# NVIDIA/DeepLearningExamples

Measured on AMD Instinct MI355X. Metric: training samples/sec, higher is better.
Workload: dtype bf16; 1 GPU; ResNet-50 v1.5 (PyTorch/Classification/ConvNets) synthetic ImageNet 224x224, label smoothing 0.1, SGD momentum 0.875 (BASELINE.json configs[1]); batch_per_gpu=256, global_batch=256, layout=NHWC, hip_graph=False, parallelism=single GPU

## Files before the change

### deeplearningexamples_amd/csrc/conv3x3.hip

```cpp
#include "gemm_tiles.h"

#define C3_MT 256

struct C3Args {
  const unsigned short* x;
  const unsigned short* w;
  unsigned short* y;
  float* stats;
  int N, H, W, CI, CO;
  int Wp, IMG, G;
  int tiles_m, tiles_n, pieces;
  FastDiv dIMG, dWp;
  const float* scale;
  const float* shift;
  const unsigned short* residual;
  int relu;
};

template <int DT, bool DGRAD, int NT, bool AFF = false>
__global__ __launch_bounds__(256, 2) void conv3x3_kernel(C3Args p) {
  constexpr int WTN = NT / 32;
  typedef Loader<DGRAD ? 1 : 0, NT, 4> LB;
  extern __shared__ __attribute__((aligned(16))) unsigned char smem_raw[];
  unsigned short* patch = (unsigned short*)smem_raw;
  unsigned short* bst = patch + p.pieces * 512;
  const int tid = threadIdx.x, lane = tid & 63, wave = tid >> 6;
  const int fr = lane & 31, fh = lane >> 5;

  int bid = blockIdx.x;
  {
    const int ntiles = p.tiles_m * p.tiles_n;
    const int q = ntiles >> 3, r = ntiles & 7, xcd = bid & 7, loc = bid >> 3;
    bid = (xcd < r ? xcd * (q + 1) : r * (q + 1) + (xcd - r) * q) + loc;
  }
  const int tm = bid / p.tiles_n, tn = bid - tm * p.tiles_n;
  const int g0 = tm * C3_MT, n0 = tn * NT;
  const int f0 = g0 - p.Wp - 1;

  ConvGeom nog;
  nog.H = nog.W = nog.C = nog.P = nog.Q = nog.R = nog.S = nog.stride = nog.Ko = 1; nog.pad = 0;
  LB lb;
  const long long ldb = 9LL * (DGRAD ? p.CO : p.CI);
  lb.init(wave, lane, n0, p.CO, ldb, nog);

  auto issue_patch = [&](int cc) __attribute__((always_inline)) {
    __amdgpu_buffer_rsrc_t rs = __builtin_amdgcn_make_buffer_rsrc((void*)p.x, 0, 0xFFFFFFE0, 0x00020000);
    for (int pc = wave; pc < p.pieces; pc += 4) {
      const int slot = pc * 8 + (lane >> 3), chunk = (lane & 7) ^ swz_kc(slot);
      const int f = f0 + slot;
      const int fc = f < 0 ? 0 : f;
      const int n = fd_div(fc, p.dIMG), rem = fc - n * p.IMG;
      const int hp = fd_div(rem, p.dWp), wp = rem - hp * p.Wp;
      const bool ok = f >= 0 && f < p.G && hp >= 1 && wp >= 1 && wp <= p.W;
      const unsigned off = (unsigned)(((((long long)n * p.H + (hp - 1)) * p.W + (wp - 1)) * p.CI + cc * 64 + chunk * 8) * 2);
      dma16(rs, patch + pc * 512, ok ? off : OOB_OFF);
    }
  };
  auto issue_b = [&](int cc, int tap, int stage) __attribute__((always_inline)) {
    const unsigned short* base = DGRAD ? p.w + (long long)cc * 64 * ldb + (8 - tap) * p.CO + n0
                                       : p.w + (long long)n0 * ldb + tap * p.CI + cc * 64;
    lb.template issue<0, LB::NP>(base, bst + stage * (NT * 64), wave, 64, 0, nog);
  };

  float16_t acc[2][WTN];
#pragma unroll
  for (int i = 0; i < 2; ++i)
#pragma unroll
    for (int j = 0; j < WTN; ++j)
#pragma unroll
      for (int r = 0; r < 16; ++r) acc[i][j][r] = 0.f;

  const int nchunks = p.CI >> 6;
  issue_patch(0);
  issue_b(0, 0, 0);
  int stage = 0;
  for (int cc = 0; cc < nchunks; ++cc) {
    if (cc > 0) {
      __syncthreads();
      issue_patch(cc);
    }
    int tapoff = 0, tapcol = 0;
    for (int tap = 0; tap < 9; ++tap) {
      __builtin_amdgcn_s_waitcnt(0x0F70);
      __syncthreads();
      if (tap < 8) issue_b(cc, tap + 1, stage ^ 1);
      else if (cc + 1 < nchunks) issue_b(cc + 1, 0, stage ^ 1);
      const unsigned short* tb = bst + stage * (NT * 64);
      int abase[2];
#pragma unroll
      for (int i = 0; i < 2; ++i) {
        const int slot = wave * 64 + i * 32 + fr + tapoff;
        abase[i] = slot * 64 + ((fh ^ swz_kc(slot)) << 3);
      }
      if constexpr (!DGRAD) {
#pragma unroll
        for (int ks = 0; ks < 4; ++ks) {
          ushort8_t fa[2], fb[WTN];
#pragma unroll
          for (int i = 0; i < 2; ++i) fa[i] = *(const ushort8_t*)(patch + (abase[i] ^ (ks << 4)));
#pragma unroll
          for (int j = 0; j < WTN; ++j) fb[j] = frag_issue<false, NT>(tb, j * 32, ks, lane);
#pragma unroll
          for (int i = 0; i < 2; ++i)
#pragma unroll
            for (int j = 0; j < WTN; ++j) acc[i][j] = Mfma32x16<DT>::run(fb[j], fa[i], acc[i][j]);
        }
      } else {
        TrPair fb[2][WTN];
#pragma unroll
        for (int j = 0; j < WTN; ++j) fb[0][j] = frag_issue<true, NT>(tb, j * 32, 0, lane);
        static_for<0, 4>([&](auto KS) __attribute__((always_inline)) {
          constexpr int ks = decltype(KS)::value, cur = ks & 1, nxt = cur ^ 1;
          ushort8_t fa[2], vb[WTN];
#pragma unroll
          for (int i = 0; i < 2; ++i) fa[i] = *(const ushort8_t*)(patch + (abase[i] ^ (ks << 4)));
          frag_wait<true>();
          if constexpr (ks < 3) {
#pragma unroll
            for (int j = 0; j < WTN; ++j) fb[nxt][j] = frag_issue<true, NT>(tb, j * 32, ks + 1, lane);
          }
#pragma unroll
          for (int j = 0; j < WTN; ++j) vb[j] = frag_value(fb[cur][j]);
#pragma unroll
          for (int i = 0; i < 2; ++i)
#pragma unroll
            for (int j = 0; j < WTN; ++j) acc[i][j] = Mfma32x16<DT>::run(vb[j], fa[i], acc[i][j]);
        });
      }
      stage ^= 1;
      if (++tapcol == 3) { tapcol = 0; tapoff += p.Wp - 2; } else ++tapoff;
    }
  }

  __syncthreads();
  constexpr int LPR = NT / 8, RPT = 64 / LPR, TRIPS = 32 / RPT, MASK = NT / 4 - 1;
  float* epi = (float*)smem_raw + wave * (32 * NT);
  const int erow = lane / LPR, ecg = lane % LPR;
  if constexpr (AFF) {
    float sc[8], sh[8];
    {
      const float4_t s0 = *(const float4_t*)(p.scale + n0 + ecg * 8), s1 = *(const float4_t*)(p.scale + n0 + ecg * 8 + 4);
      const float4_t h0 = *(const float4_t*)(p.shift + n0 + ecg * 8), h1 = *(const float4_t*)(p.shift + n0 + ecg * 8 + 4);
#pragma unroll
      for (int r = 0; r < 4; ++r) { sc[r] = s0[r]; sc[4 + r] = s1[r]; sh[r] = h0[r]; sh[4 + r] = h1[r]; }
    }
#pragma unroll
    for (int i = 0; i < 2; ++i) {
      int off[TRIPS];
      ushort8_t rv[TRIPS];
#pragma unroll
      for (int t = 0; t < TRIPS; ++t) {
        const int g = g0 + wave * 64 + i * 32 + t * RPT + erow;
        const int n = fd_div(g, p.dIMG), rem = g - n * p.IMG;
// ... 39 lines not shown
#pragma unroll
  for (int i = 0; i < 2; ++i) {
#pragma unroll
    for (int j = 0; j < WTN; ++j)
#pragma unroll
      for (int qd = 0; qd < 4; ++qd) {
        const float4_t v = {acc[i][j][qd * 4 + 0], acc[i][j][qd * 4 + 1], acc[i][j][qd * 4 + 2], acc[i][j][qd * 4 + 3]};
        const int c4 = j * 8 + qd * 2 + fh;
        *(float4_t*)(epi + fr * NT + ((c4 ^ (fr & MASK)) << 2)) = v;
      }
    asm volatile("s_waitcnt lgkmcnt(0)" ::: "memory");
#pragma unroll
    for (int t = 0; t < TRIPS; ++t) {
      const int row = t * RPT + erow;
      const float4_t lo = *(const float4_t*)(epi + row * NT + (((2 * ecg) ^ (row & MASK)) << 2));
      const float4_t hi = *(const float4_t*)(epi + row * NT + (((2 * ecg + 1) ^ (row & MASK)) << 2));
      const int g = g0 + wave * 64 + i * 32 + row;
      const int n = fd_div(g, p.dIMG), rem = g - n * p.IMG;
      const int hp = fd_div(rem, p.dWp), wp = rem - hp * p.Wp;
      const bool ok = g < p.G && hp >= 1 && wp >= 1 && wp <= p.W;
      if (ok) {
        float v[8] = {lo[0], lo[1], lo[2], lo[3], hi[0], hi[1], hi[2], hi[3]};
        const ushort8_t ov = pack8<DT>(v);
        *(ushort8_t*)(p.y + (((long long)n * p.H + (hp - 1)) * p.W + (wp - 1)) * p.CO + n0 + ecg * 8) = ov;
        if (p.stats) {
          float vr[8];
          unpack8<DT>(ov, vr);
#pragma unroll
          for (int r = 0; r < 8; ++r) { st0[r] += vr[r]; st1[r] += vr[r] * vr[r]; }
        }
      }
    }
    asm volatile("s_waitcnt lgkmcnt(0)" ::: "memory");
  }
  if (p.stats) {
#pragma unroll
    for (int r = 0; r < 8; ++r) {
#pragma unroll
      for (int o = LPR; o < 64; o <<= 1) {
        st0[r] += __shfl_xor(st0[r], o, 64);
        st1[r] += __shfl_xor(st1[r], o, 64);
      }
    }
    __syncthreads();
    float* red = (float*)smem_raw;
    if (lane < LPR) {
#pragma unroll
// ... 52 lines not shown
                               int W, int C, int Ko, int dgrad, int dtype, hipStream_t stream) {
  const int CO = dgrad ? C : Ko;
  C3Args p;
  int NT;
  size_t lds;
  if (!c3_plan(x, w, y, N, H, W, dgrad ? Ko : C, CO, dgrad, dtype, &p, &NT, &lds)) return 0;
  p.stats = stats;
  if (stats && stats_bytes < (long long)p.tiles_m * 2 * CO * 4) {
    dle_set_error("conv3x3: statistics buffer too small (%d tile rows)", p.tiles_m);
    return 2;
  }
  dim3 grid((unsigned)(p.tiles_m * p.tiles_n)), block(256);
#define C3_GO(DT, DG, NTV) DLE_LAUNCH_LDS((conv3x3_kernel<DT, DG, NTV>), grid, block, lds, stream, p)
#define C3_PICK(DT) do { if (dgrad) { if (NT == 128) C3_GO(DT, true, 128); else C3_GO(DT, true, 64); } \
                         else { if (NT == 128) C3_GO(DT, false, 128); else C3_GO(DT, false, 64); } } while (0)
  if (dtype == DLE_F16) C3_PICK(DLE_F16); else C3_PICK(DLE_BF16);
#undef C3_GO
#undef C3_PICK
  hipError_t e = hipGetLastError();
  if (e != hipSuccess) { dle_set_error("conv3x3 launch failed: %s", hipGetErrorString(e)); return (int)e + 1000; }
  return 1;
}

static long long g_c3_affine_launches = 0;
extern "C" int64_t dle_conv3x3_affine_launch_count(void) { return __atomic_load_n(&g_c3_affine_launches, __ATOMIC_RELAXED); }

extern "C" int dle_conv3x3_affine_try(const void* x, const void* w, void* y, const float* scale, const float* shift,
                                      const void* residual, int N, int H, int W, int C, int Ko, int dtype, int relu,
                                      hipStream_t stream) {
  if ((((uintptr_t)scale) | ((uintptr_t)shift) | ((uintptr_t)residual)) & 15) return 0;
  if ((long long)N * H * W * Ko >= 0x7FFFFFFFLL) return 0;
  C3Args p;
  int NT;
  size_t lds;
  if (!c3_plan(x, w, y, N, H, W, C, Ko, 0, dtype, &p, &NT, &lds)) return 0;
  p.scale = scale; p.shift = shift; p.residual = (const unsigned short*)residual; p.relu = relu;
  dim3 grid((unsigned)(p.tiles_m * p.tiles_n)), block(256);
#define C3_GO(DT, NTV) DLE_LAUNCH_LDS((conv3x3_kernel<DT, false, NTV, true>), grid, block, lds, stream, p)
#define C3_PICK(DT) do { if (NT == 128) C3_GO(DT, 128); else C3_GO(DT, 64); } while (0)
  if (dtype == DLE_F16) C3_PICK(DLE_F16); else C3_PICK(DLE_BF16);
#undef C3_GO
#undef C3_PICK
  hipError_t e = hipGetLastError();
  if (e != hipSuccess) { dle_set_error("conv3x3 affine launch failed: %s", hipGetErrorString(e)); return (int)e + 1000; }
  __atomic_fetch_add(&g_c3_affine_launches, 1, __ATOMIC_RELAXED);
  return 1;
// ... 2 lines not shown
```

### deeplearningexamples_amd/csrc/gemm_dma.hip

```cpp
#include "gemm_tiles.h"

#define SLAB_MODE(p) ((p).ws != nullptr)
#define GEMM2_LDS_BYTES (2 * (BM * BK + BN * BK) * 2)

struct Gemm2Args {
  const unsigned short* A;
  const unsigned short* B;
  void* C;
  void* aux;
  const float* bias;
  const unsigned short* mask_src;
  int M, N, K;
  long long lda, ldb, ldc;
  int out_dtype, act, splitk, accumulate;
  float alpha;
  float* ws;
  ConvGeom cg;
  int batch_inner, batch_count;
  int unused_pad;
  float* stats;
  int force_small;
  int stats_sums;
  long long row_extra;
  FastDiv row_div;
// ... 896 lines not shown
  if ((M & 255) != 0 || workspace_bytes < (long long)((M + 127) / 128) * N * 4) return 0;
  bool launched = false;
  DLE_TRY(dle_gemm8_relu_bwd_bits_try(A, B, C, bits, (float*)workspace, M, N, K, lda, ldb, dtype, stream), launched = true);
  if (!launched) return 0;
  hipLaunchKernelGGL(colsum_fold_kernel, dim3((N + 15) / 16), dim3(256), 0, stream, (const float*)workspace, colsum_out, N,
                     (M + 127) / 128, accumulate_colsum);
  hipError_t e = hipGetLastError();
  if (e != hipSuccess) { dle_set_error("colsum_fold launch failed: %s", hipGetErrorString(e)); return (int)e + 1000; }
  return 1;
}


static int conv_check(const char* what, int N, int H, int W, int C, int Ko, int R, int S, int stride, int pad,
                      int P, int Q, int dtype) {
  DLE_CHECK_ARG(dtype == DLE_F16 || dtype == DLE_BF16, "%s: 16-bit dtypes only (got %d)", what, dtype);
  DLE_CHECK_ARG(N > 0 && H > 0 && W > 0 && R > 0 && S > 0 && stride > 0 && pad >= 0, "%s: bad geometry", what);
  DLE_CHECK_ARG(C % 8 == 0 && Ko % 8 == 0, "%s: channel counts must be multiples of 8 (C=%d, K=%d)", what, C, Ko);
  DLE_CHECK_ARG(P == (H + 2 * pad - R) / stride + 1 && Q == (W + 2 * pad - S) / stride + 1, "%s: output size mismatch", what);
  DLE_CHECK_ARG((long long)N * H * W * C * 2 < 0xFFFFFFE0LL && (long long)N * P * Q * Ko * 2 < 0xFFFFFFE0LL,
                "%s: tensors above 4 GiB are not addressable by this kernel", what);
  return 0;
}

extern "C" int dle_conv2d_fwd(const void* x, const void* w, void* y, const float* bias, int N, int H, int W, int C,
                              int Ko, int R, int S, int stride, int pad, int dtype, int out_dtype, int act,
                              hipStream_t stream) {
  const int P = (H + 2 * pad - R) / stride + 1, Q = (W + 2 * pad - S) / stride + 1;
  if (int rc = conv_check("conv2d_fwd", N, H, W, C, Ko, R, S, stride, pad, P, Q, dtype)) return rc;
  DLE_CHECK_ARG(x && w && y, "conv2d_fwd: null pointer");
  DLE_CHECK_ARG(act == ACT_NONE || act == ACT_RELU, "conv2d_fwd: unsupported epilogue %d", act);
  if (R == 3 && S == 3 && stride == 1 && pad == 1 && !bias && act == ACT_NONE && out_dtype == dtype)
    DLE_TRY(dle_conv3x3_try(x, w, y, nullptr, 0, N, H, W, C, Ko, 0, dtype, stream), return 0);
  Gemm2Args p = {};
  p.A = (const unsigned short*)x; p.B = (const unsigned short*)w; p.C = y; p.bias = bias;
  p.M = N * P * Q; p.N = Ko; p.K = R * S * C; p.lda = 0; p.ldb = (long long)R * S * C; p.ldc = Ko;
  p.out_dtype = out_dtype; p.act = act; p.splitk = 1; p.accumulate = 0; p.alpha = 1.f;
  p.cg = make_geom(H, W, C, P, Q, R, S, stride, pad, Ko);
  return launch_gemm(p, dtype, 2, 0, 0, stream);
}

extern "C" int dle_conv2d_fwd_affine(const void* x, const void* w, void* y, const float* scale, const float* shift,
                                     const void* residual, int N, int H, int W, int C, int Ko, int R, int S, int stride,
                                     int pad, int dtype, int relu, hipStream_t stream) {
  DLE_CHECK_ARG(R > 0 && S > 0 && stride > 0 && pad >= 0 && H + 2 * pad >= R && W + 2 * pad >= S, "conv2d_fwd_affine: bad geometry");
  const int P = (H + 2 * pad - R) / stride + 1, Q = (W + 2 * pad - S) / stride + 1;
  if (int rc = conv_check("conv2d_fwd_affine", N, H, W, C, Ko, R, S, stride, pad, P, Q, dtype)) return rc;
  DLE_CHECK_ARG(x && w && y && scale && shift, "conv2d_fwd_affine: null pointer");
  DLE_CHECK_ARG(((((uintptr_t)x) | ((uintptr_t)w) | ((uintptr_t)y) | ((uintptr_t)scale) | ((uintptr_t)shift) | ((uintptr_t)residual)) & 15) == 0,
                "conv2d_fwd_affine: every operand must be 16-byte aligned");
  const long long M = (long long)N * P * Q;
  DLE_CHECK_ARG(M < 0x7FFFFFFFLL && (long long)R * S * C < 0x7FFFFFFFLL, "conv2d_fwd_affine: too many output pixels");
  if (R == 3 && S == 3 && stride == 1 && pad == 1)
    DLE_TRY(dle_conv3x3_affine_try(x, w, y, scale, shift, residual, N, H, W, C, Ko, dtype, relu, stream), return 0);
  const bool matrix = R == 1 && S == 1 && stride == 1 && pad == 0 && (long long)C * BM * 2 <= 0x7FFFFFFFLL;
  Gemm2Args p = {};
// ... 14 lines not shown
  if (dtype == DLE_F16) GOA(DLE_F16); else GOA(DLE_BF16);
#undef GOA
  hipError_t e = hipGetLastError();
  if (e != hipSuccess) { dle_set_error("conv2d_fwd_affine launch failed: %s", hipGetErrorString(e)); return (int)e; }
  return 0;
}

static const long long CONV_STATS_GEMM8_MAX_M = 65536;

extern "C" int dle_conv2d_fwd_colstats(const void* x, const void* w, void* y, int N, int H, int W, int C, int Ko, int R,
                                       int S, int stride, int pad, int dtype, float* col_partial,
                                       int64_t col_partial_bytes, int* groups, hipStream_t stream) {
  const int P = (H + 2 * pad - R) / stride + 1, Q = (W + 2 * pad - S) / stride + 1;
  if (int rc = conv_check("conv2d_fwd_colstats", N, H, W, C, Ko, R, S, stride, pad, P, Q, dtype)) return rc;
  DLE_CHECK_ARG(x && w && y && col_partial && groups, "conv2d_fwd_colstats: null pointer");
  DLE_CHECK_ARG((((uintptr_t)y) & 15) == 0, "conv2d_fwd_colstats: output must be 16-byte aligned");
  const long long M = (long long)N * P * Q;
  const int g = (int)((M + BM - 1) / BM);
  DLE_CHECK_ARG(col_partial_bytes >= (long long)g * 2 * Ko * 4, "conv2d_fwd_colstats: partial buffer too small (%lld tile rows)", (long long)g);
  *groups = g;
  if (R == 3 && S == 3 && stride == 1 && pad == 1 && col_partial_bytes >= (long long)dle_conv3x3_tiles(N, H, W) * 2 * Ko * 4)
    DLE_TRY(dle_conv3x3_try(x, w, y, col_partial, col_partial_bytes, N, H, W, C, Ko, 0, dtype, stream),
            *groups = (int)(((long long)N * (H + 1) * (W + 2) + 255) / 256); return 0);
  const bool plain = R == 1 && S == 1 && stride == 1 && pad == 0;
  if (plain && M < 0x7FFFFFFF && (M & 255) == 0 && M <= CONV_STATS_GEMM8_MAX_M && C >= 128 && Ko >= 256)
    DLE_TRY(dle_gemm8_colstats_try(x, w, y, (int)M, Ko, C, C, C, Ko, dtype, col_partial, stream), *groups = g; return 0);
  if (plain && M < 0x7FFFFFFF) {
    static const int kmin = dle_env_int("DLE_EXPAND_STATS_KMIN", 64);
    const int eg = dle_gemm_expand_groups((int)M, Ko, C);
    if (dle_gemm_expand_enabled() && C >= kmin && col_partial_bytes >= (long long)eg * 2 * Ko * 4)
      DLE_TRY(dle_gemm_expand_try(x, w, y, nullptr, nullptr, col_partial, (int)M, Ko, C, C, C, Ko, 1, dtype, dtype, EX_ACT_NONE, stream),
              *groups = eg; return 0);
  }
  Gemm2Args p = {};
  p.A = (const unsigned short*)x; p.B = (const unsigned short*)w; p.C = y;
  p.M = (int)M; p.N = Ko; p.K = R * S * C; p.ldb = (long long)R * S * C; p.ldc = Ko;
  p.out_dtype = dtype; p.act = ACT_NONE; p.splitk = 1; p.accumulate = 0; p.alpha = 1.f;
  p.stats = col_partial; p.force_small = 1;
  p.lda = plain ? C : 0;
  p.cg = make_geom(H, W, C, P, Q, R, S, stride, pad, Ko);
  return launch_gemm(p, dtype, plain ? 0 : 2, 0, 0, stream);
}

extern "C" int dle_conv2d_dgrad(const void* dy, const void* w, void* dx, const void* addend, int N, int H, int W,
                                int C, int Ko, int R, int S, int stride, int pad, int dtype, hipStream_t stream) {
  const int P = (H + 2 * pad - R) / stride + 1, Q = (W + 2 * pad - S) / stride + 1;
  if (int rc = conv_check("conv2d_dgrad", N, H, W, C, Ko, R, S, stride, pad, P, Q, dtype)) return rc;
  DLE_CHECK_ARG(dy && w && dx, "conv2d_dgrad: null pointer");
  if (R == 3 && S == 3 && stride == 1 && pad == 1 && !addend)
    DLE_TRY(dle_conv3x3_try(dy, w, dx, nullptr, 0, N, H, W, C, Ko, 1, dtype, stream), return 0);
  Gemm2Args p = {};
  p.A = (const unsigned short*)dy; p.B = (const unsigned short*)w; p.C = dx;
  p.mask_src = (const unsigned short*)addend;
  p.M = N * H * W; p.N = C; p.K = R * S * Ko; p.lda = 0; p.ldb = 0; p.ldc = C;
  p.out_dtype = dtype; p.act = addend ? ACT_ADD : ACT_NONE; p.splitk = 1; p.accumulate = 0; p.alpha = 1.f;
// ... 45 lines not shown
                                                            int Ko, int C) {
  const long long total = 9LL * Ko * C;
  for (long long i = (long long)blockIdx.x * blockDim.x + threadIdx.x; i < total; i += (long long)gridDim.x * blockDim.x) {
    const int c = (int)(i % C);
    const long long t = i / C;
    const int rs = (int)(t % 9), ko = (int)(t / 9);
    const int r = rs / 3, sx = rs - r * 3;
    const int a = r == 1 ? 0 : 1, b = sx == 1 ? 0 : 1;
    const int rp = r == 0 ? 1 : 0, sp = sx == 0 ? 1 : 0;
    const int Sp = b ? 2 : 1, taps = (a ? 2 : 1) * Sp;
    const long long base = (long long)C * Ko * (a == 0 ? (b == 0 ? 0 : 1) : (b == 0 ? 3 : 5));
    out[base + ((long long)c * taps + rp * Sp + sp) * Ko + ko] = w[i];
  }
}

extern "C" int dle_conv2d_dgrad_s2(const void* dy, const void* w, void* dx, int N, int H, int W, int C, int Ko,
                                   void* workspace, int64_t workspace_bytes, int dtype, hipStream_t stream) {
  DLE_CHECK_ARG(dtype == DLE_F16 || dtype == DLE_BF16, "conv2d_dgrad_s2: 16-bit dtypes only");
  DLE_CHECK_ARG(dy && w && dx && workspace, "conv2d_dgrad_s2: null pointer");
  DLE_CHECK_ARG(N > 0 && H > 0 && W > 0 && (H & 1) == 0 && (W & 1) == 0, "conv2d_dgrad_s2: H, W must be even");
  DLE_CHECK_ARG(C % 8 == 0 && Ko % 64 == 0, "conv2d_dgrad_s2: C a multiple of 8, Ko a multiple of 64 (got %d, %d)", C, Ko);
  DLE_CHECK_ARG(workspace_bytes >= 9LL * Ko * C * 2 && (((uintptr_t)workspace) & 15) == 0, "conv2d_dgrad_s2: workspace too small");
  DLE_CHECK_ARG((long long)N * H * W * C * 2 < 0xFFFFFFE0LL, "conv2d_dgrad_s2: tensors above 4 GiB are not addressable");
  const int P = H / 2, Q = W / 2;
  {
    long long g = (9LL * Ko * C + 255) / 256;
    if (g > 2048) g = 2048;
    if (dtype == DLE_F16) hipLaunchKernelGGL(dgrad_s2_pack_kernel<DLE_F16>, dim3((unsigned)g), dim3(256), 0, stream, (const unsigned short*)w, (unsigned short*)workspace, Ko, C);
    else hipLaunchKernelGGL(dgrad_s2_pack_kernel<DLE_BF16>, dim3((unsigned)g), dim3(256), 0, stream, (const unsigned short*)w, (unsigned short*)workspace, Ko, C);
    DLE_LAUNCH_CHECK();
  }
  static const int cls_off[4] = {0, 1, 3, 5};
  for (int a = 0; a < 2; ++a)
    for (int b = 0; b < 2; ++b) {
      const int Rp = a ? 2 : 1, Sp = b ? 2 : 1;
      Gemm2Args p = {};
      p.A = (const unsigned short*)dy;
      p.B = (const unsigned short*)workspace + (long long)C * Ko * cls_off[2 * a + b];
      p.C = (unsigned short*)dx + ((long long)a * W + b) * C;
      p.M = N * P * Q; p.N = C; p.K = Rp * Sp * Ko; p.lda = 0; p.ldb = (long long)Rp * Sp * Ko;
      p.ldc = 2LL * C;
      p.row_extra = (long long)W * C;
      p.row_div = make_fastdiv(Q);
      p.out_dtype = dtype; p.act = ACT_NONE; p.splitk = 1; p.accumulate = 0; p.alpha = 1.f;
      p.cg = make_geom(P, Q, Ko, P, Q, Rp, Sp, 1, 0, C);
      if (int rc = launch_gemm(p, dtype, 2, 0, 0, stream)) return rc;
// ... 28 lines not shown
```

### deeplearningexamples_amd/csrc/gemm_expand.hip

```cpp
#include "gemm_tiles.h"

#define EX_TN 128
#define EX_PAD 8

struct ExpandArgs {
  const unsigned short* A;
  const unsigned short* B;
  unsigned short* C;
  const unsigned short* src;
  const unsigned char* bits;
  float* stats;
  int M, N, K;
  long long lda, ldb, ldc;
  int b_kc, row_tiles, groups, col_tiles;
  FastDiv dHW, dW;
  int up_HW, up_W, up_P, up_Q;
  long long ld_src;
  const unsigned short* t2;
  const unsigned char* bits2;
  const float* mean2;
  const float* rstd2;
};

template <int DT> struct ExMfma;
template <> struct ExMfma<DLE_F16> {
  static __device__ __forceinline__ float4_t run(ushort8_t a, ushort8_t b, float4_t c) {
    return __builtin_amdgcn_mfma_f32_16x16x32_f16(__builtin_bit_cast(half8_t, a), __builtin_bit_cast(half8_t, b), c, 0, 0, 0);
  }
};
template <> struct ExMfma<DLE_BF16> {
  static __device__ __forceinline__ float4_t run(ushort8_t a, ushort8_t b, float4_t c) {
    return __builtin_amdgcn_mfma_f32_16x16x32_bf16(__builtin_bit_cast(bf16x8_t, a), __builtin_bit_cast(bf16x8_t, b), c, 0, 0, 0);
  }
};

__device__ __forceinline__ int ex_pos(int nl) {
  const int j = nl >> 5, r = nl & 31;
  return 32 * j + 16 * ((r >> 2) & 1) + 4 * (r >> 3) + (r & 3);
}

template <int KS, int ACT, bool BRED = false>
struct ExStream {
  ushort8_t fa[KS];
  ushort8_t sv[ACT ? 4 : 1];
  ushort8_t tv[BRED ? 4 : 1];
  uint4_t mb;
  uint4_t mb2;
  long long o0;
  bool live;
  bool has;
  __device__ __forceinline__ void load_a(const ExpandArgs& p, int m, int kg) {
    const long long mr = m < p.M ? m : p.M - 1;
    const unsigned short* arow = p.A + mr * p.lda + kg * 8;
#pragma unroll
    for (int ks = 0; ks < KS; ++ks) fa[ks] = *(const ushort8_t*)(arow + ks * 32);
  }
  __device__ __forceinline__ void load_src(const ExpandArgs& p, int m, int n0, int kg) {
    live = m < p.M;
    const long long mr = live ? m : p.M - 1;
    o0 = mr * p.ldc + n0 + kg * 8;
    if (ACT == 3) {
      const int mi = (int)mr;
      const int n = fd_div(mi, p.dHW), rem = mi - n * p.up_HW;
      const int h = fd_div(rem, p.dW), w = rem - h * p.up_W;
      has = !((h | w) & 1);
      const long long cr = has ? ((long long)n * p.up_P + (h >> 1)) * p.up_Q + (w >> 1) : 0;
      const unsigned short* srow = p.src + cr * p.ld_src + n0 + kg * 8;
#pragma unroll
      for (int j = 0; j < 4; ++j) sv[j] = *(const ushort8_t*)(srow + 32 * j);
    } else if (ACT) {
#pragma unroll
      for (int j = 0; j < 4; ++j) sv[j] = *(const ushort8_t*)(p.src + o0 + 32 * j);
    }
    if (ACT == 2) mb = *(const uint4_t*)(p.bits + ((mr * p.ldc + n0) >> 3));
    if (BRED) {
// ... 9 lines not shown
  const bool h8 = fr & 8, h4 = fr & 4, h2 = fr & 2, h1 = fr & 1;
#pragma unroll
  for (int q = 0; q < 16; ++q) {
    const float keep = h8 ? v[16 + q] : v[q], send = h8 ? v[q] : v[16 + q];
    w16[q] = keep + __shfl_xor(send, 8, 64);
  }
#pragma unroll
  for (int q = 0; q < 8; ++q) {
    const float keep = h4 ? w16[8 + q] : w16[q], send = h4 ? w16[q] : w16[8 + q];
    w8[q] = keep + __shfl_xor(send, 4, 64);
  }
#pragma unroll
  for (int q = 0; q < 4; ++q) {
    const float keep = h2 ? w8[4 + q] : w8[q], send = h2 ? w8[q] : w8[4 + q];
    w4[q] = keep + __shfl_xor(send, 2, 64);
  }
#pragma unroll
  for (int q = 0; q < 2; ++q) {
    const float keep = h1 ? w4[2 + q] : w4[q], send = h1 ? w4[q] : w4[2 + q];
    acc[q] += keep + __shfl_xor(send, 1, 64);
  }
}

template <int DT, int KS, int ACT, bool STATS, int NW, bool BRED = false>
__global__ __launch_bounds__(NW * 64) __attribute__((amdgpu_waves_per_eu((STATS || BRED) ? 3 : 4)))
void gemm_expand_kernel(ExpandArgs p) {
  constexpr int K = KS * 32, LDW = K + EX_PAD, TM = NW * 16;
  extern __shared__ __attribute__((aligned(16))) unsigned char smem_raw[];
  unsigned short* wl = (unsigned short*)smem_raw;
  const int lane = threadIdx.x & 63, wave = threadIdx.x >> 6;
  const int fr = lane & 15, kg = lane >> 4;
  const int xcd = blockIdx.x & 7, slot = blockIdx.x >> 3;
  const int tn = slot % p.col_tiles, g = (slot / p.col_tiles) * 8 + xcd;
  const int n0 = tn * EX_TN;
  if (p.b_kc) {
    constexpr int CPR = K / 8;
    for (int c = threadIdx.x; c < EX_TN * CPR; c += NW * 64) {
      const int nl = c / CPR, kc = c - nl * CPR;
      const ushort8_t v = *(const ushort8_t*)(p.B + (long long)(n0 + nl) * p.ldb + kc * 8);
      *(ushort8_t*)(wl + ex_pos(nl) * LDW + kc * 8) = v;
    }
  } else {
    for (int c = threadIdx.x; c < K * (EX_TN / 8); c += NW * 64) {
      const int k = c >> 4, nc = c & 15;
      const ushort8_t v = *(const ushort8_t*)(p.B + (long long)k * p.ldb + n0 + nc * 8);
#pragma unroll
      for (int e = 0; e < 8; ++e) wl[ex_pos(nc * 8 + e) * LDW + k] = v[e];
    }
  }
  float* mu2 = (float*)(smem_raw + EX_TN * LDW * 2);
  if (BRED) {
    for (int c = threadIdx.x; c < EX_TN; c += NW * 64) { mu2[c] = p.mean2[n0 + c]; mu2[EX_TN + c] = p.rstd2[n0 + c]; }
  }
  __syncthreads();
  float s1[STATS ? 32 : 1], s2[STATS ? 32 : 1];
  if (STATS) {
#pragma unroll
    for (int i = 0; i < 32; ++i) { s1[i] = 0.f; s2[i] = 0.f; }
  }
  float b1[2] = {0.f, 0.f}, b2s[2] = {0.f, 0.f};
  const unsigned short* wrow = wl + fr * LDW + kg * 8;
  const int mrow = wave * 16 + fr;
  ExStream<KS, ACT, BRED> cur;
  cur.load_a(p, g * TM + mrow, kg);
  cur.load_src(p, g * TM + mrow, n0, kg);
  for (int tm = g; tm < p.row_tiles; tm += p.groups) {
    const int m_next = (tm + p.groups) * TM + mrow;
    float4_t acc[8];
#pragma unroll
    for (int b = 0; b < 8; ++b) acc[b] = (float4_t){0.f, 0.f, 0.f, 0.f};
#pragma unroll
    for (int ks = 0; ks < KS; ++ks) {
#pragma unroll
      for (int b = 0; b < 8; ++b) {
        const ushort8_t fw = *(const ushort8_t*)(wrow + b * 16 * LDW + ks * 32);
        acc[b] = ExMfma<DT>::run(fw, cur.fa[ks], acc[b]);
      }
      __builtin_amdgcn_sched_barrier(0);
    }
    cur.load_a(p, m_next, kg);
    ushort8_t outv[4];
    float tg[BRED ? 32 : 1], tx[BRED ? 32 : 1];
    const bool live_cur = cur.live;
    const bool has_cur = ACT == 3 ? cur.has : true;
#pragma unroll
    for (int j = 0; j < 4; ++j) {
// ... 147 lines not shown
  do {                                                                                                                   \
    constexpr int NW_ = KS > 4 ? 8 : 4;                                                                                  \
    DLE_LAUNCH_LDS((gemm_expand_kernel<DT, KS, ACT, ST, NW_>), grid, block, lds_bytes, stream, p);                       \
  } while (0)
#define PICK_ACT(DT, KS)                                              \
  do {                                                                \
    if (stats) { if (act != EX_ACT_NONE) return 0; GO(DT, KS, EX_ACT_NONE, true); } \
    else if (act == EX_ACT_NONE) GO(DT, KS, EX_ACT_NONE, false);                    \
    else if (act == EX_ACT_ADD) GO(DT, KS, EX_ACT_ADD, false);                      \
    else GO(DT, KS, EX_ACT_ADD_MASKED, false);                                      \
  } while (0)
#define PICK_K(DT)                                   \
  do {                                               \
    if (K == 64) PICK_ACT(DT, 2);                    \
    else if (K == 128) PICK_ACT(DT, 4);              \
    else PICK_ACT(DT, 8);                            \
  } while (0)
  if (in_dtype == DLE_F16) PICK_K(DLE_F16); else PICK_K(DLE_BF16);
#undef PICK_K
#undef PICK_ACT
#undef GO
  hipError_t e = hipGetLastError();
  if (e != hipSuccess) { dle_set_error("gemm_expand launch failed: %s", hipGetErrorString(e)); return (int)e + 1000; }
  return 1;
}

extern "C" int dle_gemm_expand_masked_bnred(const void* A, const void* B, void* C, const void* src, const void* bits, const void* t2,
                                            const void* bits2, const float* mean2, const float* rstd2, float* partial,
                                            int64_t partial_bytes, int M, int N, int K, int64_t lda, int64_t ldb, int64_t ldc,
                                            int b_kc, int dtype, hipStream_t stream) {
  if (!dle_gemm_expand_enabled()) return 0;
  const int k256 = dle_env_int("DLE_GEMM_BNRED_K256", 0);
  if (M < 4096 || (K != 64 && K != 128 && !(K == 256 && k256)) || (N % EX_TN) != 0 || N < 2 * K) return 0;
  if (dtype != DLE_F16 && dtype != DLE_BF16) return 0;
  if (!A || !B || !C || !src || !bits || !t2 || !bits2 || !mean2 || !rstd2 || !partial) return 0;
  if (((((uintptr_t)A) | ((uintptr_t)B) | ((uintptr_t)C) | ((uintptr_t)src) | ((uintptr_t)t2) | ((uintptr_t)bits) | ((uintptr_t)bits2)) & 15) != 0 ||
      (lda & 7) || (ldb & 7) || (ldc % EX_TN) != 0)
    return 0;
  ExpandArgs p = {(const unsigned short*)A, (const unsigned short*)B, (unsigned short*)C, (const unsigned short*)src,
                  (const unsigned char*)bits, partial, M, N, K, (long long)lda, (long long)ldb, (long long)ldc, b_kc, 0, 0, 0};
  p.t2 = (const unsigned short*)t2; p.bits2 = (const unsigned char*)bits2; p.mean2 = mean2; p.rstd2 = rstd2;
  const int tmr = ex_rows_per_tile(K);
  p.row_tiles = (M + tmr - 1) / tmr;
  p.col_tiles = N / EX_TN;
  p.groups = dle_gemm_expand_groups(M, N, K);
  if (partial_bytes < (long long)p.groups * 2 * N * 4) return 0;
// ... 50 lines not shown
```

### deeplearningexamples_amd/csrc/gemm_family.h

```cpp
#pragma once
#include "common.h"

#define BM 128
#define BN 128
#define BK 64

enum { ACT_NONE = DLE_ACT_NONE, ACT_RELU = DLE_ACT_RELU, ACT_GELU = DLE_ACT_GELU, ACT_RELU_BWD = DLE_ACT_RELU_BWD,
       ACT_ADD = DLE_ACT_ADD, ACT_GELU_BWD = DLE_ACT_GELU_BWD, ACT_TANH = DLE_ACT_TANH, ACT_TANH_BWD = DLE_ACT_TANH_BWD,
       ACT_ADD_MASKED = DLE_ACT_ADD_MASKED,
       ACT_MUL = DLE_ACT_MUL,
       ACT_GELU_DAUX = DLE_ACT_GELU_DAUX,
       ACT_LAST_PUBLIC = DLE_ACT_GELU_DAUX,
       ACT_RELU_BITS = 11, ACT_RELU_BWD_BITS = 12,
       ACT_ADD_RELU = 13 };

inline bool act_needs_src(int act) {
  return act == ACT_RELU_BWD || act == ACT_ADD || act == ACT_GELU_BWD || act == ACT_TANH_BWD || act == ACT_ADD_MASKED || act == ACT_MUL ||
         act == ACT_ADD_RELU;
}

enum { EX_ACT_NONE = 0, EX_ACT_ADD = 1, EX_ACT_ADD_MASKED = 2 };
inline int expand_act_kind(int act) { return act == ACT_NONE ? EX_ACT_NONE : act == ACT_ADD ? EX_ACT_ADD : EX_ACT_ADD_MASKED; }

inline bool dle_gemm_expand_enabled() { return dle_env_int("DLE_GEMM_EXPAND", 1) != 0; }
// ... 14 lines not shown
  const float th = fast_tanh(k0 * (x + k1 * x2 * x));
  const float hp = 0.5f * (1.0f + th);
  d = hp + 0.5f * x * (1.f - th * th) * k0 * (1.f + 3.f * k1 * x2);
  return x * hp;
}

extern "C" {
int dle_gemm_dma_try(const void* A, const void* B, void* C, void* aux, const float* bias, const void* mask_src, int M, int N, int K,
                     int64_t lda, int64_t ldb, int64_t ldc, int a_kc, int b_kc, int in_dtype, int out_dtype, int act, int splitk,
                     int accumulate, float alpha, void* workspace, int64_t workspace_bytes, hipStream_t stream);
int dle_gemm8_try(const void* A, const void* B, void* C, void* aux, const float* bias, const void* src, int M, int N, int K,
                  int64_t lda, int64_t ldb, int64_t ldc, int a_kc, int b_kc, int in_dtype, int out_dtype, int act, int splitk,
                  int accumulate, float alpha, float* ws, float* stats, hipStream_t stream);
int dle_gemm8_colstats_try(const void* A, const void* B, void* C, int M, int N, int K, int64_t lda, int64_t ldb, int64_t ldc,
                           int dtype, float* stats, hipStream_t stream);
int dle_gemm8_relu_bwd_bits_try(const void* dY, const void* W, void* dX, const void* bits, float* colsum_partial, int M, int N,
                                int K, int64_t lddy, int64_t ldw, int dtype, hipStream_t stream);
int dle_gemm_smallm_try(const void* A, const void* B, void* C, const float* bias, const void* src, int M, int N, int K, int64_t lda,
                        int64_t ldb, int64_t ldc, int in_dtype, int out_dtype, int act_add, int accumulate, float alpha,
                        hipStream_t stream);
int dle_gemm_expand_try(const void* A, const void* B, void* C, const void* src, const void* bits, float* stats, int M, int N, int K,
                        int64_t lda, int64_t ldb, int64_t ldc, int b_kc, int in_dtype, int out_dtype, int act, hipStream_t stream);
int dle_gemm_expand_groups(int M, int N, int K);
int dle_conv3x3_try(const void* x, const void* w, void* y, float* stats, long long stats_bytes, int N, int H, int W, int C, int Ko,
                    int dgrad, int dtype, hipStream_t stream);
int dle_conv3x3_tiles(int N, int H, int W);
int dle_conv3x3_affine_try(const void* x, const void* w, void* y, const float* scale, const float* shift, const void* residual, int N,
                           int H, int W, int C, int Ko, int dtype, int relu, hipStream_t stream);
int dle_conv3x3_wgrad_try(const void* dy, const void* x, float* dw, int N, int H, int W, int C, int Ko, int dtype, int accumulate,
                          void* workspace, int64_t workspace_bytes, hipStream_t stream);
}
int gemm_regs_launch(const void* A, const void* B, void* C, void* aux, const float* bias, const void* mask_src, int M, int N, int K,
                     int64_t lda, int64_t ldb, int64_t ldc, int a_kc, int b_kc, int in_dtype, int out_dtype, int act, int splitk,
                     int accumulate, float alpha, hipStream_t stream);
hipError_t wgrad1x1_fold(const float* ws, float* dw, long long total4, int G, int accumulate, hipStream_t stream);
```

Baseline: 13230 samples/s.

## Add strided-2 conv3x3 fwd/dgrad via parity-plane decomposition and strided 1x1 expand GEMM

Extends the implicit-GEMM conv3x3 kernel with a stride-2 mode. The forward pass walks the four input parity planes, each with its subset of taps. The dgrad pass splits the output by parity class, so each block runs only the 1, 2 or 4 taps that apply to it. A strided 1x1 forward path is added to the expand GEMM by remapping A rows to every other pixel, which avoids the generic GEMM and any gather copy. The intent is to move ResNet's downsampling convolutions off slower generic paths onto the tuned MFMA kernels. The cost is more template instances, heavier address arithmetic, and uneven per-block work in dgrad.

```diff
diff --git a/deeplearningexamples_amd/csrc/conv3x3.hip b/deeplearningexamples_amd/csrc/conv3x3.hip
--- a/deeplearningexamples_amd/csrc/conv3x3.hip
+++ b/deeplearningexamples_amd/csrc/conv3x3.hip
@@ -17,7 +17,7 @@
   int relu;
 };
 
-template <int DT, bool DGRAD, int NT, bool AFF = false>
+template <int DT, bool DGRAD, int NT, bool AFF = false, bool S2 = false>
 __global__ __launch_bounds__(256, 2) void conv3x3_kernel(C3Args p) {
   constexpr int WTN = NT / 32;
   typedef Loader<DGRAD ? 1 : 0, NT, 4> LB;
@@ -28,6 +28,12 @@
   const int fr = lane & 31, fh = lane >> 5;
 
   int bid = blockIdx.x;
+  int ca = 0, cb = 0;
+  if constexpr (S2 && DGRAD) {
+    const int ntiles = p.tiles_m * p.tiles_n, ord = bid / ntiles;
+    bid -= ord * ntiles;
+    ca = (3 - ord) >> 1; cb = (3 - ord) & 1;
+  }
   {
     const int ntiles = p.tiles_m * p.tiles_n;
     const int q = ntiles >> 3, r = ntiles & 7, xcd = bid & 7, loc = bid >> 3;
@@ -35,7 +41,7 @@
   }
   const int tm = bid / p.tiles_n, tn = bid - tm * p.tiles_n;
   const int g0 = tm * C3_MT, n0 = tn * NT;
-  const int f0 = g0 - p.Wp - 1;
+  const int f0 = S2 && DGRAD ? g0 : g0 - p.Wp - 1;
 
   ConvGeom nog;
   nog.H = nog.W = nog.C = nog.P = nog.Q = nog.R = nog.S = nog.stride = nog.Ko = 1; nog.pad = 0;
@@ -56,11 +62,35 @@
       dma16(rs, patch + pc * 512, ok ? off : OOB_OFF);
     }
   };
+  auto issue_plane = [&](int cc, int a, int b) __attribute__((always_inline)) {
+    __amdgpu_buffer_rsrc_t rs = __builtin_amdgcn_make_buffer_rsrc((void*)p.x, 0, 0xFFFFFFE0, 0x00020000);
+    for (int pc = wave; pc < p.pieces; pc += 4) {
+      const int slot = pc * 8 + (lane >> 3), chunk = (lane & 7) ^ swz_kc(slot);
+      const int f = f0 + slot;
+      const int fc = f < 0 ? 0 : f;
+      const int n = fd_div(fc, p.dIMG), rem = fc - n * p.IMG;
+      const int hp = fd_div(rem, p.dWp), wp = rem - hp * p.Wp;
+      const bool ok = f >= 0 && f < p.G && hp >= 1 && wp >= 1 && wp <= p.W;
+      const long long pix = ((long long)n * (2 * p.H) + (2 * (hp - 1) + a)) * (2 * p.W) + (2 * (wp - 1) + b);
+      const unsigned off = (unsigned)((pix * p.CI + cc * 64 + chunk * 8) * 2);
+      dma16(rs, patch + pc * 512, ok ? off : OOB_OFF);
+    }
+  };
   auto issue_b = [&](int cc, int tap, int stage) __attribute__((always_inline)) {
     const unsigned short* base = DGRAD ? p.w + (long long)cc * 64 * ldb + (8 - tap) * p.CO + n0
                                        : p.w + (long long)n0 * ldb + tap * p.CI + cc * 64;
     lb.template issue<0, LB::NP>(base, bst + stage * (NT * 64), wave, 64, 0, nog);
   };
+  auto issue_b_s2d = [&](int cc, int tap, int stage) __attribute__((always_inline)) {
+    lb.template issue<0, LB::NP>(p.w + (long long)cc * 64 * ldb + tap * p.CO + n0, bst + stage * (NT * 64), wave, 64, 0, nog);
+  };
+  auto s2_tap = [&](int a, int b, int t, int& widx, int& off) __attribute__((always_inline)) {
+    const int ri = b ? t >> 1 : t, si = b ? t & 1 : 0;
+    const int r = a ? 2 * ri : 1, s = b ? 2 * si : 1;
+    widx = r * 3 + s;
+    const int sh = (r == 0 ? p.Wp : 0) + (s == 0 ? 1 : 0);
+    off = DGRAD ? sh : p.Wp + 1 - sh;
+  };
 
   float16_t acc[2][WTN];
 #pragma unroll
@@ -71,20 +101,9 @@
       for (int r = 0; r < 16; ++r) acc[i][j][r] = 0.f;
 
   const int nchunks = p.CI >> 6;
-  issue_patch(0);
-  issue_b(0, 0, 0);
   int stage = 0;
-  for (int cc = 0; cc < nchunks; ++cc) {
-    if (cc > 0) {
-      __syncthreads();
-      issue_patch(cc);
-    }
-    int tapoff = 0, tapcol = 0;
-    for (int tap = 0; tap < 9; ++tap) {
-      __builtin_amdgcn_s_waitcnt(0x0F70);
-      __syncthreads();
-      if (tap < 8) issue_b(cc, tap + 1, stage ^ 1);
-      else if (cc + 1 < nchunks) issue_b(cc + 1, 0, stage ^ 1);
+  if constexpr (S2) {
+    auto mma_tap = [&](int tapoff) __attribute__((always_inline)) {
       const unsigned short* tb = bst + stage * (NT * 64);
       int abase[2];
 #pragma unroll
@@ -128,7 +147,107 @@
         });
       }
       stage ^= 1;
-      if (++tapcol == 3) { tapcol = 0; tapoff += p.Wp - 2; } else ++tapoff;
+    };
+    int widx, off;
+    if constexpr (DGRAD) {
+      const int ntap = (ca + 1) * (cb + 1);
+      issue_patch(0);
+      s2_tap(ca, cb, 0, widx, off);
+      issue_b_s2d(0, widx, 0);
+      for (int cc = 0; cc < nchunks; ++cc) {
+        if (cc > 0) {
+          __syncthreads();
+          issue_patch(cc);
+        }
+        for (int t = 0; t < ntap; ++t) {
+          __builtin_amdgcn_s_waitcnt(0x0F70);
+          __syncthreads();
+          if (t + 1 < ntap) { s2_tap(ca, cb, t + 1, widx, off); issue_b_s2d(cc, widx, stage ^ 1); }
+          else if (cc + 1 < nchunks) { s2_tap(ca, cb, 0, widx, off); issue_b_s2d(cc + 1, widx, stage ^ 1); }
+          s2_tap(ca, cb, t, widx, off);
+          mma_tap(off);
+        }
+      }
+    } else {
+      issue_plane(0, 0, 0);
+      issue_b(0, 4, 0);
+      for (int cc = 0; cc < nchunks; ++cc)
+        for (int pl = 0; pl < 4; ++pl) {
+          const int a = pl >> 1, b = pl & 1, ntap = (a + 1) * (b + 1);
+          if (cc + pl > 0) {
+            __syncthreads();
+            issue_plane(cc, a, b);
+          }
+          for (int t = 0; t < ntap; ++t) {
+            __builtin_amdgcn_s_waitcnt(0x0F70);
+            __syncthreads();
+            if (t + 1 < ntap) { s2_tap(a, b, t + 1, widx, off); issue_b(cc, widx, stage ^ 1); }
+            else if (pl < 3) { s2_tap((pl + 1) >> 1, (pl + 1) & 1, 0, widx, off); issue_b(cc, widx, stage ^ 1); }
+            else if (cc + 1 < nchunks) issue_b(cc + 1, 4, stage ^ 1);
+            s2_tap(a, b, t, widx, off);
+            mma_tap(off);
+          }
+        }
+    }
+  } else {
+    issue_patch(0);
+    issue_b(0, 0, 0);
+    for (int cc = 0; cc < nchunks; ++cc) {
+      if (cc > 0) {
+        __syncthreads();
+        issue_patch(cc);
+      }
+      int tapoff = 0, tapcol = 0;
+      for (int tap = 0; tap < 9; ++tap) {
+        __builtin_amdgcn_s_waitcnt(0x0F70);
+        __syncthreads();
+        if (tap < 8) issue_b(cc, tap + 1, stage ^ 1);
+        else if (cc + 1 < nchunks) issue_b(cc + 1, 0, stage ^ 1);
+        const unsigned short* tb = bst + stage * (NT * 64);
+        int abase[2];
+#pragma unroll
+        for (int i = 0; i < 2; ++i) {
+          const int slot = wave * 64 + i * 32 + fr + tapoff;
+          abase[i] = slot * 64 + ((fh ^ swz_kc(slot)) << 3);
+        }
+        if constexpr (!DGRAD) {
+#pragma unroll
+          for (int ks = 0; ks < 4; ++ks) {
+            ushort8_t fa[2], fb[WTN];
+#pragma unroll
+            for (int i = 0; i < 2; ++i) fa[i] = *(const ushort8_t*)(patch + (abase[i] ^ (ks << 4)));
+#pragma unroll
+            for (int j = 0; j < WTN; ++j) fb[j] = frag_issue<false, NT>(tb, j * 32, ks, lane);
+#pragma unroll
+            for (int i = 0; i < 2; ++i)
+#pragma unroll
+              for (int j = 0; j < WTN; ++j) acc[i][j] = Mfma32x16<DT>::run(fb[j], fa[i], acc[i][j]);
+          }
+        } else {
+          TrPair fb[2][WTN];
+#pragma unroll
+          for (int j = 0; j < WTN; ++j) fb[0][j] = frag_issue<true, NT>(tb, j * 32, 0, lane);
+          static_for<0, 4>([&](auto KS) __attribute__((always_inline)) {
+            constexpr int ks = decltype(KS)::value, cur = ks & 1, nxt = cur ^ 1;
+            ushort8_t fa[2], vb[WTN];
+#pragma unroll
+            for (int i = 0; i < 2; ++i) fa[i] = *(const ushort8_t*)(patch + (abase[i] ^ (ks << 4)));
+            frag_wait<true>();
+            if constexpr (ks < 3) {
+#pragma unroll
+              for (int j = 0; j < WTN; ++j) fb[nxt][j] = frag_issue<true, NT>(tb, j * 32, ks + 1, lane);
+            }
+#pragma unroll
+            for (int j = 0; j < WTN; ++j) vb[j] = frag_value(fb[cur][j]);
+#pragma unroll
+            for (int i = 0; i < 2; ++i)
+#pragma unroll
+              for (int j = 0; j < WTN; ++j) acc[i][j] = Mfma32x16<DT>::run(vb[j], fa[i], acc[i][j]);
+          });
+        }
+        stage ^= 1;
+        if (++tapcol == 3) { tapcol = 0; tapoff += p.Wp - 2; } else ++tapoff;
+      }
     }
   }
 
@@ -214,7 +333,10 @@
       if (ok) {
         float v[8] = {lo[0], lo[1], lo[2], lo[3], hi[0], hi[1], hi[2], hi[3]};
         const ushort8_t ov = pack8<DT>(v);
-        *(ushort8_t*)(p.y + (((long long)n * p.H + (hp - 1)) * p.W + (wp - 1)) * p.CO + n0 + ecg * 8) = ov;
+        long long pix;
+        if constexpr (S2 && DGRAD) pix = ((long long)n * (2 * p.H) + (2 * (hp - 1) + ca)) * (2 * p.W) + (2 * (wp - 1) + cb);
+        else pix = ((long long)n * p.H + (hp - 1)) * p.W + (wp - 1);
+        *(ushort8_t*)(p.y + pix * p.CO + n0 + ecg * 8) = ov;
         if (p.stats) {
           float vr[8];
           unpack8<DT>(ov, vr);
@@ -313,6 +435,57 @@
   return 1;
 }
 
+static bool c3_plan_s2(const void* big, const void* w, const void* small, int N, int H, int W, int CI, int CO, long long big_ch,
+                       int dtype, C3Args* p, int* nt, size_t* lds) {
+  if ((H & 1) || (W & 1) || H < 2 || W < 2) return false;
+  if ((((uintptr_t)big) | ((uintptr_t)small)) & 15) return false;
+  if ((long long)N * H * W * big_ch * 2 >= 0xFFFFFFE0LL) return false;
+  if (!c3_plan(big, w, small, N, H / 2, W / 2, CI, CO, 1, dtype, p, nt, lds)) return false;
+  p->pieces = (C3_MT + p->Wp + 2 + 7) / 8;
+  size_t need = (size_t)p->pieces * 1024 + 2 * (size_t)*nt * 64 * 2;
+  const size_t epi = 4 * 32 * (size_t)*nt * 4;
+  *lds = need > epi ? need : epi;
+  return true;
+}
+
+extern "C" int dle_conv3x3_dgrad_s2_try(const void* dy, const void* w, void* dx, int N, int H, int W, int C, int Ko, int dtype,
+                                        hipStream_t stream) {
+  C3Args p;
+  int NT;
+  size_t lds;
+  if (!c3_plan_s2(dx, w, dy, N, H, W, Ko, C, C, dtype, &p, &NT, &lds)) return 0;
+  p.x = (const unsigned short*)dy; p.y = (unsigned short*)dx;
+  if ((long long)N * (H / 2) * (W / 2) * Ko * 2 >= 0xFFFFFFE0LL || 4LL * p.tiles_m * p.tiles_n >= 0x7FFFFFFFLL) return 0;
+  dim3 grid((unsigned)(4 * p.tiles_m * p.tiles_n)), block(256);
+#define C3_GO(DT, NTV) DLE_LAUNCH_LDS((conv3x3_kernel<DT, true, NTV, false, true>), grid, block, lds, stream, p)
+#define C3_PICK(DT) do { if (NT == 128) C3_GO(DT, 128); else C3_GO(DT, 64); } while (0)
+  if (dtype == DLE_F16) C3_PICK(DLE_F16); else C3_PICK(DLE_BF16);
+#undef C3_GO
+#undef C3_PICK
+  hipError_t e = hipGetLastError();
+  if (e != hipSuccess) { dle_set_error("conv3x3 dgrad_s2 launch failed: %s", hipGetErrorString(e)); return (int)e + 1000; }
+  return 1;
+}
+
+extern "C" int dle_conv3x3_fwd_s2_try(const void* x, const void* w, void* y, float* stats, long long stats_bytes, int N, int H,
+                                      int W, int C, int Ko, int dtype, hipStream_t stream) {
+  C3Args p;
+  int NT;
+  size_t lds;
+  if (!c3_plan_s2(x, w, y, N, H, W, C, Ko, C, dtype, &p, &NT, &lds)) return 0;
+  if (stats && stats_bytes < (long long)p.tiles_m * 2 * Ko * 4) return 0;
+  p.stats = stats;
+  dim3 grid((unsigned)(p.tiles_m * p.tiles_n)), block(256);
+#define C3_GO(DT, NTV) DLE_LAUNCH_LDS((conv3x3_kernel<DT, false, NTV, false, true>), grid, block, lds, stream, p)
+#define C3_PICK(DT) do { if (NT == 128) C3_GO(DT, 128); else C3_GO(DT, 64); } while (0)
+  if (dtype == DLE_F16) C3_PICK(DLE_F16); else C3_PICK(DLE_BF16);
+#undef C3_GO
+#undef C3_PICK
+  hipError_t e = hipGetLastError();
+  if (e != hipSuccess) { dle_set_error("conv3x3 fwd_s2 launch failed: %s", hipGetErrorString(e)); return (int)e + 1000; }
+  return 1;
+}
+
 static long long g_c3_affine_launches = 0;
 extern "C" int64_t dle_conv3x3_affine_launch_count(void) { return __atomic_load_n(&g_c3_affine_launches, __ATOMIC_RELAXED); }
 
diff --git a/deeplearningexamples_amd/csrc/gemm_dma.hip b/deeplearningexamples_amd/csrc/gemm_dma.hip
--- a/deeplearningexamples_amd/csrc/gemm_dma.hip
+++ b/deeplearningexamples_amd/csrc/gemm_dma.hip
@@ -942,6 +942,8 @@
   return 0;
 }
 
+static bool conv3x3_s2_fwd_routed(int P, int Q, int C) { return P * Q >= 100 && C >= 256; }
+
 extern "C" int dle_conv2d_fwd(const void* x, const void* w, void* y, const float* bias, int N, int H, int W, int C,
                               int Ko, int R, int S, int stride, int pad, int dtype, int out_dtype, int act,
                               hipStream_t stream) {
@@ -951,6 +953,8 @@
   DLE_CHECK_ARG(act == ACT_NONE || act == ACT_RELU, "conv2d_fwd: unsupported epilogue %d", act);
   if (R == 3 && S == 3 && stride == 1 && pad == 1 && !bias && act == ACT_NONE && out_dtype == dtype)
     DLE_TRY(dle_conv3x3_try(x, w, y, nullptr, 0, N, H, W, C, Ko, 0, dtype, stream), return 0);
+  if (R == 3 && S == 3 && stride == 2 && pad == 1 && !bias && act == ACT_NONE && out_dtype == dtype && conv3x3_s2_fwd_routed(P, Q, C))
+    DLE_TRY(dle_conv3x3_fwd_s2_try(x, w, y, nullptr, 0, N, H, W, C, Ko, dtype, stream), return 0);
   Gemm2Args p = {};
   p.A = (const unsigned short*)x; p.B = (const unsigned short*)w; p.C = y; p.bias = bias;
   p.M = N * P * Q; p.N = Ko; p.K = R * S * C; p.lda = 0; p.ldb = (long long)R * S * C; p.ldc = Ko;
@@ -1011,6 +1015,9 @@
   if (R == 3 && S == 3 && stride == 1 && pad == 1 && col_partial_bytes >= (long long)dle_conv3x3_tiles(N, H, W) * 2 * Ko * 4)
     DLE_TRY(dle_conv3x3_try(x, w, y, col_partial, col_partial_bytes, N, H, W, C, Ko, 0, dtype, stream),
             *groups = (int)(((long long)N * (H + 1) * (W + 2) + 255) / 256); return 0);
+  if (R == 3 && S == 3 && stride == 2 && pad == 1 && conv3x3_s2_fwd_routed(P, Q, C))
+    DLE_TRY(dle_conv3x3_fwd_s2_try(x, w, y, col_partial, col_partial_bytes, N, H, W, C, Ko, dtype, stream),
+            *groups = dle_conv3x3_tiles(N, P, Q); return 0);
   const bool plain = R == 1 && S == 1 && stride == 1 && pad == 0;
   if (plain && M < 0x7FFFFFFF && (M & 255) == 0 && M <= CONV_STATS_GEMM8_MAX_M && C >= 128 && Ko >= 256)
     DLE_TRY(dle_gemm8_colstats_try(x, w, y, (int)M, Ko, C, C, C, Ko, dtype, col_partial, stream), *groups = g; return 0);
@@ -1020,6 +1027,11 @@
     if (dle_gemm_expand_enabled() && C >= kmin && col_partial_bytes >= (long long)eg * 2 * Ko * 4)
       DLE_TRY(dle_gemm_expand_try(x, w, y, nullptr, nullptr, col_partial, (int)M, Ko, C, C, C, Ko, 1, dtype, dtype, EX_ACT_NONE, stream),
               *groups = eg; return 0);
+  }
+  if (R == 1 && S == 1 && stride == 2 && pad == 0 && M < 0x7FFFFFFF && dle_gemm_expand_enabled()) {
+    const int eg = dle_gemm_expand_groups((int)M, Ko, C);
+    if (col_partial_bytes >= (long long)eg * 2 * Ko * 4)
+      DLE_TRY(dle_gemm_expand_s2_try(x, w, y, col_partial, N, H, W, C, Ko, dtype, stream), *groups = eg; return 0);
   }
   Gemm2Args p = {};
   p.A = (const unsigned short*)x; p.B = (const unsigned short*)w; p.C = y;
@@ -1111,6 +1123,7 @@
   DLE_CHECK_ARG(C % 8 == 0 && Ko % 64 == 0, "conv2d_dgrad_s2: C a multiple of 8, Ko a multiple of 64 (got %d, %d)", C, Ko);
   DLE_CHECK_ARG(workspace_bytes >= 9LL * Ko * C * 2 && (((uintptr_t)workspace) & 15) == 0, "conv2d_dgrad_s2: workspace too small");
   DLE_CHECK_ARG((long long)N * H * W * C * 2 < 0xFFFFFFE0LL, "conv2d_dgrad_s2: tensors above 4 GiB are not addressable");
+  DLE_TRY(dle_conv3x3_dgrad_s2_try(dy, w, dx, N, H, W, C, Ko, dtype, stream), return 0);
   const int P = H / 2, Q = W / 2;
   {
     long long g = (9LL * Ko * C + 255) / 256;
diff --git a/deeplearningexamples_amd/csrc/gemm_expand.hip b/deeplearningexamples_amd/csrc/gemm_expand.hip
--- a/deeplearningexamples_amd/csrc/gemm_expand.hip
+++ b/deeplearningexamples_amd/csrc/gemm_expand.hip
@@ -39,7 +39,7 @@
   return 32 * j + 16 * ((r >> 2) & 1) + 4 * (r >> 3) + (r & 3);
 }
 
-template <int KS, int ACT, bool BRED = false>
+template <int KS, int ACT, bool BRED = false, bool AS2 = false>
 struct ExStream {
   ushort8_t fa[KS];
   ushort8_t sv[ACT ? 4 : 1];
@@ -50,7 +50,13 @@
   bool live;
   bool has;
   __device__ __forceinline__ void load_a(const ExpandArgs& p, int m, int kg) {
-    const long long mr = m < p.M ? m : p.M - 1;
+    long long mr = m < p.M ? m : p.M - 1;
+    if (AS2) {
+      const int mi = (int)mr;
+      const int n = fd_div(mi, p.dHW), rem = mi - n * p.up_HW;
+      const int pp = fd_div(rem, p.dW), q = rem - pp * p.up_W;
+      mr = ((long long)n * p.up_P + 2 * pp) * p.up_Q + 2 * q;
+    }
     const unsigned short* arow = p.A + mr * p.lda + kg * 8;
 #pragma unroll
     for (int ks = 0; ks < KS; ++ks) fa[ks] = *(const ushort8_t*)(arow + ks * 32);
@@ -106,7 +112,7 @@
   }
 }
 
-template <int DT, int KS, int ACT, bool STATS, int NW, bool BRED = false>
+template <int DT, int KS, int ACT, bool STATS, int NW, bool BRED = false, bool AS2 = false>
 __global__ __launch_bounds__(NW * 64) __attribute__((amdgpu_waves_per_eu((STATS || BRED) ? 3 : 4)))
 void gemm_expand_kernel(ExpandArgs p) {
   constexpr int K = KS * 32, LDW = K + EX_PAD, TM = NW * 16;
@@ -145,7 +151,7 @@
   float b1[2] = {0.f, 0.f}, b2s[2] = {0.f, 0.f};
   const unsigned short* wrow = wl + fr * LDW + kg * 8;
   const int mrow = wave * 16 + fr;
-  ExStream<KS, ACT, BRED> cur;
+  ExStream<KS, ACT, BRED, AS2> cur;
   cur.load_a(p, g * TM + mrow, kg);
   cur.load_src(p, g * TM + mrow, n0, kg);
   for (int tm = g; tm < p.row_tiles; tm += p.groups) {
@@ -339,6 +345,38 @@
 #undef GO
   hipError_t e = hipGetLastError();
   if (e != hipSuccess) { dle_set_error("gemm_expand launch failed: %s", hipGetErrorString(e)); return (int)e + 1000; }
+  return 1;
+}
+
+extern "C" int dle_gemm_expand_s2_try(const void* x, const void* w, void* y, float* stats, int N, int H, int W, int K, int Nc,
+                                      int dtype, hipStream_t stream) {
+  if (N <= 0 || H <= 0 || W <= 0 || (H & 1) || (W & 1) || !stats) return 0;
+  if ((K != 64 && K != 128 && K != 256) || (Nc % EX_TN) != 0 || Nc < 2 * K || (dtype != DLE_F16 && dtype != DLE_BF16)) return 0;
+  if (((((uintptr_t)x) | ((uintptr_t)w) | ((uintptr_t)y)) & 15) != 0) return 0;
+  const int P = H / 2, Q = W / 2;
+  const long long M = (long long)N * P * Q;
+  if (M >= 0x7FFFFFFFLL - 65536 * 128) return 0;
+  ExpandArgs p = {(const unsigned short*)x, (const unsigned short*)w, (unsigned short*)y, nullptr, nullptr, stats, (int)M, Nc, K,
+                  (long long)K, (long long)K, (long long)Nc, 1, 0, 0, 0};
+  p.dHW = make_fastdiv(P * Q); p.dW = make_fastdiv(Q);
+  p.up_HW = P * Q; p.up_W = Q; p.up_P = H; p.up_Q = W;
+  const int tmr = ex_rows_per_tile(K);
+  p.row_tiles = (int)((M + tmr - 1) / tmr);
+  p.col_tiles = Nc / EX_TN;
+  p.groups = dle_gemm_expand_groups((int)M, Nc, K);
+  const int lds_bytes = EX_TN * (K + EX_PAD) * 2 > 8 * 2 * EX_TN * 4 ? EX_TN * (K + EX_PAD) * 2 : 8 * 2 * EX_TN * 4;
+  const dim3 grid((unsigned)(p.groups * p.col_tiles)), block(tmr * 4);
+#define GO(DT, KS)                                                                                                       \
+  do {                                                                                                                   \
+    constexpr int NW_ = KS > 4 ? 8 : 4;                                                                                  \
+    DLE_LAUNCH_LDS((gemm_expand_kernel<DT, KS, EX_ACT_NONE, true, NW_, false, true>), grid, block, lds_bytes, stream, p); \
+  } while (0)
+#define PICK_K(DT) do { if (K == 64) GO(DT, 2); else if (K == 128) GO(DT, 4); else GO(DT, 8); } while (0)
+  if (dtype == DLE_F16) PICK_K(DLE_F16); else PICK_K(DLE_BF16);
+#undef PICK_K
+#undef GO
+  hipError_t e = hipGetLastError();
+  if (e != hipSuccess) { dle_set_error("gemm_expand_s2 launch failed: %s", hipGetErrorString(e)); return (int)e + 1000; }
   return 1;
 }
 
diff --git a/deeplearningexamples_amd/csrc/gemm_family.h b/deeplearningexamples_amd/csrc/gemm_family.h
--- a/deeplearningexamples_amd/csrc/gemm_family.h
+++ b/deeplearningexamples_amd/csrc/gemm_family.h
@@ -60,9 +60,14 @@
 int dle_gemm_expand_try(const void* A, const void* B, void* C, const void* src, const void* bits, float* stats, int M, int N, int K,
                         int64_t lda, int64_t ldb, int64_t ldc, int b_kc, int in_dtype, int out_dtype, int act, hipStream_t stream);
 int dle_gemm_expand_groups(int M, int N, int K);
+int dle_gemm_expand_s2_try(const void* x, const void* w, void* y, float* stats, int N, int H, int W, int K, int Nc, int dtype,
+                           hipStream_t stream);
 int dle_conv3x3_try(const void* x, const void* w, void* y, float* stats, long long stats_bytes, int N, int H, int W, int C, int Ko,
                     int dgrad, int dtype, hipStream_t stream);
 int dle_conv3x3_tiles(int N, int H, int W);
+int dle_conv3x3_fwd_s2_try(const void* x, const void* w, void* y, float* stats, long long stats_bytes, int N, int H, int W, int C,
+                           int Ko, int dtype, hipStream_t stream);
+int dle_conv3x3_dgrad_s2_try(const void* dy, const void* w, void* dx, int N, int H, int W, int C, int Ko, int dtype, hipStream_t stream);
 int dle_conv3x3_affine_try(const void* x, const void* w, void* y, const float* scale, const float* shift, const void* residual, int N,
                            int H, int W, int C, int Ko, int dtype, int relu, hipStream_t stream);
 int dle_conv3x3_wgrad_try(const void* dy, const void* x, float* dw, int N, int H, int W, int C, int Ko, int dtype, int accumulate,
```

Result: no change. 13330 samples/s, median of 4 (+0.7%).
